# caiyuanhao1998/Open-DiffusionGS

Hardware: AMD Instinct MI355X
Metric: novel-view renders/sec (DiT step + GS raster) at 256^2 (higher is better)
Workload: dtype bf16; 1 GPU; obj-256 sampling step (BASELINE.json configs[2]): DGSDenoiser.forward = DiT image_to_gaussians (width 1024, 24 blocks, L=4098, bf16 MFMA, fp32 accumulate) + 4 fp32 rasterizations of P=262146 Gaussians at 256^2 per sample; random-init weights; batch_per_gpu=1, views=4, resolution=256, gaussians=262146, parallelism=dp1

## Files before the change

### open-diffusiongs_amd/csrc/raster_forward.hip

```cpp
#include <string.h>

#include "raster_cells.h"

namespace dgs {

struct FwdParams {
    int P, D, M, W, H, V, vps, gx, gy, T;
    const float *bg, *means3D, *shs, *colors_pre, *opac, *scales, *rots, *cov_pre, *viewm, *projm, *campos, *tanfov;
    float tanfovx, tanfovy, scale_mod;
    int prefiltered, raw_act;
    int bin_mode;
    int bitonic_cap;
    int bitonic_any;
    int exact_exp;
    int debug;
    int* radii;
    float* out_color;
    float *out_depth, *out_alpha;
    GeomState g;
    ImageState im;
    BinningState bn;
};

__device__ __forceinline__ void view_tanfov(const FwdParams& p, int v, float* tx, float* ty) {
// ... 21 lines not shown
                        -0.4570457994644658f * y * (4.0f * zz - xx - yy) * SH(11) +
                        0.3731763325901154f * z * (2.0f * zz - 3.0f * xx - 3.0f * yy) * SH(12) +
                        -0.4570457994644658f * x * (4.0f * zz - xx - yy) * SH(13) + 1.445305721320277f * z * (xx - yy) * SH(14) +
                        -0.5900435899266435f * x * (xx - 3.0f * yy) * SH(15);
                }
            }
        }
#undef SH
        r += 0.5f;
        if (r < 0) bits |= 1u << c;
        out[c] = fmaxf(r, 0.0f);
    }
    *clamp_bits = bits;
}

__device__ __forceinline__ bool preprocess_one(const FwdParams& p, int v, int idx, int* rx0, int* ry0, int* rx1, int* ry1, uint32_t* depth_key) {
    const int s = v / p.vps;
    const size_t gi = (size_t)v * p.P + idx;
    const size_t si = (size_t)s * p.P + idx;
    p.radii[gi] = 0;
    p.g.tiles_touched[gi] = 0;
    p.g.keys[0][gi] = 0xFFFFFFFFu;
    const float* vm = p.viewm + 16 * v;
    const float* pm = p.projm + 16 * v;
    const float mx = p.means3D[3 * si], my = p.means3D[3 * si + 1], mz = p.means3D[3 * si + 2];
    const float hx = pm[0] * mx + pm[4] * my + pm[8] * mz + pm[12];
    const float hy = pm[1] * mx + pm[5] * my + pm[9] * mz + pm[13];
    const float hw = pm[3] * mx + pm[7] * my + pm[11] * mz + pm[15];
    const float pw = 1.0f / (hw + 0.0000001f);
    const float projx = hx * pw, projy = hy * pw;
    float tx = vm[0] * mx + vm[4] * my + vm[8] * mz + vm[12];
    float ty = vm[1] * mx + vm[5] * my + vm[9] * mz + vm[13];
    const float tz = vm[2] * mx + vm[6] * my + vm[10] * mz + vm[14];
    if (tz <= 0.2f) {
        if (p.prefiltered) p.im.totals[1] = DGS_ERR_PREFILTERED_CULLED;
        return false;
    }
// ... 45 lines not shown
        sh_to_rgb(p.D, p.shs + 3 * (size_t)p.M * si, mx - cam[0], my - cam[1], mz - cam[2], rgb, &cbits);
    }
    float op = p.opac[si];
    if (p.raw_act) op = 1.0f / (1.0f + det_expf(-op));
    const float cut = (op > 0.0f) ? (__logf(1.0f / (255.0f * op)) - 0.004f) : __builtin_inff();
    p.g.depths[gi] = tz;
    p.radii[gi] = irad;
    p.g.means2D[gi] = make_float2(px, py);
    BlendRecord* rec = p.g.blend + gi;
    rec->co = make_float4(conx, cony, conz, op);
    rec->rc = make_float4(rgb[0], rgb[1], rgb[2], cut);
    *reinterpret_cast<float4*>(&rec->xy) = make_float4(px, py, tz, 0.f);
    p.g.clamped[gi] = (uint8_t)cbits;
    p.g.tiles_touched[gi] = (uint32_t)((y1 - y0) * (x1 - x0));
    p.g.keys[0][gi] = __float_as_uint(tz);
    *depth_key = __float_as_uint(tz);
    *rx0 = x0; *ry0 = y0; *rx1 = x1; *ry1 = y1;
    return true;
}

template <bool LDS_HIST>
__global__ __launch_bounds__(256) void preprocess_kernel(FwdParams p) {
    DGS_DYNAMIC_LDS(smem);
    uint32_t* lhist = reinterpret_cast<uint32_t*>(smem);
    const int v = blockIdx.y;
    const int idx = blockIdx.x * 256 + threadIdx.x;
    if (LDS_HIST) {
        for (int i = threadIdx.x; i < p.T; i += 256) lhist[i] = 0;
        __syncthreads();
    }
    if (blockIdx.x == 0) {
        uint32_t* w = p.g.range_ws + (size_t)v * range_ws_stride(p.P);
        for (int i = threadIdx.x; i <= kRangeBuckets; i += 256) w[i] = 0u;
    }
    int x0 = 0, y0 = 0, x1 = 0, y1 = 0;
    bool vis = false;
    uint32_t depth_key = 0xFFFFFFFFu;
    if (idx < p.P) vis = preprocess_one(p, v, idx, &x0, &y0, &x1, &y1, &depth_key);
    {
        __shared__ uint32_t s_rng[2][4];
        const uint32_t key = vis ? depth_key : 0xFFFFFFFFu;
        uint32_t hi = key != 0xFFFFFFFFu ? key : 0u, lo_c = key != 0xFFFFFFFFu ? ~key : 0u;
#pragma unroll
        for (int o = 32; o > 0; o >>= 1) { hi = max(hi, (uint32_t)__shfl_xor((int)hi, o)); lo_c = max(lo_c, (uint32_t)__shfl_xor((int)lo_c, o)); }
        if ((threadIdx.x & 63) == 0) { s_rng[0][threadIdx.x >> 6] = hi; s_rng[1][threadIdx.x >> 6] = lo_c; }
        __syncthreads();
        if (threadIdx.x < 2) {
            const uint32_t m = max(max(s_rng[threadIdx.x][0], s_rng[threadIdx.x][1]), max(s_rng[threadIdx.x][2], s_rng[threadIdx.x][3]));
            if (m) atomicMax(p.im.depth_range + ((size_t)threadIdx.x * p.V + v) * kRangeSlots + (blockIdx.x % kRangeSlots), m);
        }
    }
    uint32_t* gcount = p.im.tile_count + (size_t)v * p.T;
    if (vis) {
        uint32_t* const grid = LDS_HIST ? lhist : gcount;
        atomicAdd(&grid[y0 * p.gx + x0], 1u);
        if (x1 < p.gx) atomicAdd(&grid[y0 * p.gx + x1], 0xffffffffu);
        if (y1 < p.gy) {
            atomicAdd(&grid[y1 * p.gx + x0], 0xffffffffu);
            if (x1 < p.gx) atomicAdd(&grid[y1 * p.gx + x1], 1u);
        }
    }
    if (LDS_HIST) {
        __syncthreads();
        for (int i = threadIdx.x; i < p.T; i += 256) {
            const uint32_t c = lhist[i];
            if (c) atomicAdd(&gcount[i], c);
        }
    }
}

__global__ __launch_bounds__(256) void radix_hist_kernel(const uint32_t* keys, uint32_t* hist, int P, int NB, int shift) {
    __shared__ uint32_t h[256];
    const int v = blockIdx.y, b = blockIdx.x;
    h[threadIdx.x] = 0;
    __syncthreads();
    const uint32_t* k = keys + (size_t)v * P;
    const int base = b * kSortTile;
#pragma unroll 4
// ... 53 lines not shown
        const uint32_t rank_in_wave = (uint32_t)__popcll(peers & lt_mask);
        if (valid && rank_in_wave == 0) wcount[wave][dig] = (uint32_t)__popcll(peers);
        __syncthreads();
        if (valid) {
            uint32_t pos = running[dig] + rank_in_wave;
            for (int w = 0; w < wave; ++w) pos += wcount[w][dig];
            keys_out[vo + pos] = key;
            vals_out[vo + pos] = val;
            if (rank_of) rank_of[vo + val] = pos;
        }
        __syncthreads();
        running[tid] += wcount[0][tid] + wcount[1][tid] + wcount[2][tid] + wcount[3][tid];
    }
}

struct RangeMap {
    uint32_t lo; float scale; bool any;
    __device__ __forceinline__ uint32_t bucket(uint32_t key) const { return min((uint32_t)((float)(key - lo) * scale), (uint32_t)kRangeBuckets - 1u); }
};
__device__ __forceinline__ RangeMap range_map(const uint32_t* depth_range, int V, int v, uint32_t* s_map ) {
    if (threadIdx.x < 64) {
        const int which = threadIdx.x >> 5, slot = threadIdx.x & 31;
        uint32_t x = slot < kRangeSlots ? depth_range[((size_t)which * V + v) * kRangeSlots + slot] : 0u;
#pragma unroll
        for (int o = 16; o > 0; o >>= 1) x = max(x, (uint32_t)__shfl_xor((int)x, o));
        if (slot == 0) s_map[which] = x;
    }
    __syncthreads();
    const uint32_t hi_w = s_map[0], lo_w = s_map[1];
    const uint32_t hi = hi_w, lo = ~lo_w;
// ... 19 lines not shown
        const int i = b * kRangeTile + r * 256 + tid;
        if (i < P) {
            const uint32_t key = k[i];
            if (key != 0xFFFFFFFFu) atomicAdd(&h[m.bucket(key)], 1u); else ++culled;
        }
    }
#pragma unroll
    for (int o = 32; o > 0; o >>= 1) culled += (uint32_t)__shfl_xor((int)culled, o);
    if ((tid & 63) == 0) s_c[tid >> 6] = culled;
    __syncthreads();
    uint32_t* w = ws + (size_t)v * stride;
    for (int i = tid; i < kRangeBuckets; i += 256) { const uint32_t c = h[i]; if (c) atomicAdd(&w[i], c); }
    if (tid == 0) w[2 * kRangeBuckets + 1 + b] = (s_c[0] + s_c[1]) + (s_c[2] + s_c[3]);
}

__global__ __launch_bounds__(1024) void range_plan_kernel(uint32_t* ws, int NB, int NWIN, int stride) {
    __shared__ uint32_t scratch[20];
    __shared__ uint32_t s_start[kRangeBuckets + 1];
    uint32_t* w = ws + (size_t)blockIdx.x * stride;
    const int tid = threadIdx.x;
    const uint32_t c = tid < kRangeBuckets ? w[tid] : 0u;
    uint32_t nvis;
    const uint32_t ex = block_exclusive_scan<1024>(c, scratch, &nvis);
    __syncthreads();
    if (tid < kRangeBuckets) { w[tid] = ex; w[kRangeBuckets + 1 + tid] = 0u; s_start[tid] = ex; }
    if (tid == 0) { w[kRangeBuckets] = nvis; s_start[kRangeBuckets] = nvis; }
    __syncthreads();
    for (int j = tid; j <= NWIN; j += 1024) {
        const uint32_t want = (uint32_t)j * (uint32_t)kRangeWindow;
        int lo = 0, hi = kRangeBuckets;
        while (lo < hi) { const int mid = (lo + hi) >> 1; if (s_start[mid] < want) lo = mid + 1; else hi = mid; }
        w[2 * kRangeBuckets + 1 + NB + j] = j == NWIN ? nvis : s_start[lo];
    }
    const uint32_t cc = tid < NB ? w[2 * kRangeBuckets + 1 + tid] : 0u;
    uint32_t all;
    const uint32_t cex = block_exclusive_scan<1024>(cc, scratch, &all);
    if (tid < NB) w[2 * kRangeBuckets + 1 + tid] = nvis + cex;
}

__global__ __launch_bounds__(256) void range_scatter_kernel(const uint32_t* keys, const uint32_t* depth_range, uint32_t* ws, uint32_t* keys_out,
                                                           uint32_t* vals_out, uint32_t* order, uint32_t* rank_of, int P, int V, int stride) {
    __shared__ uint32_t h[kRangeBuckets];
    __shared__ uint32_t s_cc[kRangeItems][4];
    __shared__ uint32_t s_map[2];
    const int v = blockIdx.y, b = blockIdx.x, tid = threadIdx.x, lane = tid & 63, wave = tid >> 6;
    const RangeMap m = range_map(depth_range, V, v, s_map);
    const size_t vo = (size_t)v * P;
    uint32_t* w = ws + (size_t)v * stride;
    for (int i = tid; i < kRangeBuckets; i += 256) h[i] = 0;
    __syncthreads();
    uint32_t key[kRangeItems], slot[kRangeItems];
    const unsigned long long lt_mask = (lane == 0) ? 0ull : (~0ull >> (64 - lane));
#pragma unroll
    for (int r = 0; r < kRangeItems; ++r) {
        const int i = b * kRangeTile + r * 256 + tid;
        key[r] = i < P ? keys[vo + i] : 0u;
// ... 4 lines not shown
        if (lane == 0) s_cc[r][wave] = (uint32_t)__popcll(cm);
    }
    __syncthreads();
    {
        constexpr int Q = kRangeBuckets / 256;
        uint32_t c[Q], st0[Q], got[Q];
#pragma unroll
        for (int q = 0; q < Q; ++q) { c[q] = h[tid + 256 * q]; st0[q] = w[tid + 256 * q]; }
#pragma unroll
        for (int q = 0; q < Q; ++q) got[q] = c[q] ? atomicAdd(&w[kRangeBuckets + 1 + tid + 256 * q], c[q]) : 0u;
#pragma unroll
        for (int q = 0; q < Q; ++q) h[tid + 256 * q] = st0[q] + got[q];
    }
    __syncthreads();
    const uint32_t cbase = w[2 * kRangeBuckets + 1 + b];
#pragma unroll
    for (int r = 0; r < kRangeItems; ++r) {
        const int i = b * kRangeTile + r * 256 + tid;
        if (i >= P) continue;
        if (key[r] != 0xFFFFFFFFu) {
            const uint32_t pos = h[m.bucket(key[r])] + slot[r];
            keys_out[vo + pos] = key[r];
            vals_out[vo + pos] = (uint32_t)i;
        } else {
            uint32_t off = 0;
            for (int q = 0; q < r; ++q) off += (s_cc[q][0] + s_cc[q][1]) + (s_cc[q][2] + s_cc[q][3]);
            for (int q = 0; q < wave; ++q) off += s_cc[r][q];
            const uint32_t pos = cbase + off + slot[r];
            order[vo + pos] = (uint32_t)i;
            rank_of[vo + i] = pos;
        }
    }
}

__global__ __launch_bounds__(1024) void scan_tiles_kernel(uint32_t* count, uint2* ranges, uint32_t* cursor, int n,
                                                         int32_t* totals, long long capacity, uint32_t* order, int gx, int gy,
                                                         int32_t* stats_dev, int32_t* stats_host) {
    __shared__ uint32_t scratch[20];
    __shared__ uint32_t smax;
    __shared__ uint32_t s_class[1024];
    {
        const int T = gx * gy, V = n / T;
        for (int r = threadIdx.x; r < V * gy; r += 1024) {
            uint32_t* row = count + (size_t)(r / gy) * T + (size_t)(r % gy) * gx;
            uint32_t run = 0;
            for (int x0 = 0; x0 < gx; x0 += 16) {
                uint32_t c[16];
#pragma unroll
                for (int u = 0; u < 16; ++u) c[u] = x0 + u < gx ? row[x0 + u] : 0u;
#pragma unroll
                for (int u = 0; u < 16; ++u)
                    if (x0 + u < gx) { run += c[u]; row[x0 + u] = run; }
            }
        }
        __syncthreads();
        for (int cidx = threadIdx.x; cidx < V * gx; cidx += 1024) {
            uint32_t* col = count + (size_t)(cidx / gx) * T + (cidx % gx);
            uint32_t run = 0;
            for (int y0 = 0; y0 < gy; y0 += 16) {
                uint32_t c[16];
#pragma unroll
                for (int u = 0; u < 16; ++u) c[u] = y0 + u < gy ? col[(size_t)(y0 + u) * gx] : 0u;
#pragma unroll
                for (int u = 0; u < 16; ++u)
                    if (y0 + u < gy) { run += c[u]; col[(size_t)(y0 + u) * gx] = run; }
            }
        }
        __syncthreads();
    }
    uint32_t carry = 0, mx = 0;
    if (threadIdx.x == 0) smax = 0;
    for (int base = 0; base < n; base += 1024) {
        const int i = base + threadIdx.x;
        const uint32_t c = (i < n) ? count[i] : 0u;
        mx = max(mx, c);
        uint32_t tot;
        const uint32_t ex = block_exclusive_scan<1024>(c, scratch, &tot);
        if (i < n) { ranges[i] = make_uint2(carry + ex, carry + ex + c); cursor[i] = 0; }
        carry += tot;
    }
    __syncthreads();
    atomicMax(&smax, mx);
    __syncthreads();
    if (threadIdx.x == 0) {
        totals[0] = (int32_t)carry;
        totals[2] = (int32_t)smax;
        if (capacity >= 0 && (long long)carry > capacity) totals[1] = DGS_ERR_BINNING_OVERFLOW;
        const int32_t st1 = totals[1];
        if (stats_dev) { stats_dev[0] = (int32_t)carry; stats_dev[1] = st1; stats_dev[2] = (int32_t)smax; stats_dev[3] = 1; }
        if (stats_host) {
            stats_host[0] = (int32_t)carry; stats_host[1] = st1; stats_host[2] = (int32_t)smax;
            __threadfence_system();
            *reinterpret_cast<volatile int32_t*>(stats_host + 3) = 1;
        }
    }
    deal_tiles(count, n, smax, order, s_class, scratch);
}

enum { kFormRankSort = 1, kFormScan = 2, kFormBitonic = 3 };
__host__ __device__ __forceinline__ int binning_form_of(int bin_mode, int bitonic_cap, long long num_rendered, long long longest,
                                                        long long T, long long P, long long V, bool any_len = false) {
    const bool fits = bitonic_cap > 0 && (any_len || longest <= bitonic_cap);
    if (bin_mode == kFormScan || bin_mode == kFormRankSort) return bin_mode;
    if (bin_mode == kFormBitonic) return fits ? kFormBitonic : kFormRankSort;
    if (num_rendered * 10 >= T * P * V) return kFormScan;
    return fits ? kFormBitonic : kFormRankSort;
}
__host__ __device__ __forceinline__ bool scan_form_possible(int gx, int gy, long long T, long long P) {
    return gx <= 255 && gy <= 255 && T * P <= (1ll << 31);
}
__device__ __forceinline__ int binning_form(const FwdParams& p) {
    return binning_form_of(p.bin_mode, p.bitonic_cap, (long long)(uint32_t)p.im.totals[0], (long long)(uint32_t)p.im.totals[2], p.T, p.P, p.V,
                           p.bitonic_any != 0);
}
__device__ __forceinline__ bool binning_is_scan(const FwdParams& p) { return binning_form(p) == kFormScan; }

template <bool LDS_AGG>
__global__ __launch_bounds__(256) void emit_instances_kernel(FwdParams p) {
    DGS_DYNAMIC_LDS(smem);
    uint32_t* lcnt = reinterpret_cast<uint32_t*>(smem);
    uint32_t* lbase = lcnt + p.T;
    const int form = binning_form(p);
    if (p.im.totals[1] != 0 || form == kFormScan) return;
    const bool wide = form == kFormBitonic;
    const int v = blockIdx.y;
// ... 256 lines not shown
    }
    {
        uint32_t m = 8 * NT;
        while (m < n) m <<= 1;
        for (uint32_t i = n + tid; i < m; i += NT) keys[i] = ~0ull;
        __syncthreads();
        bitonic_sort_lds<NT>(keys, m, tid);
    }
    __syncthreads();
    for (uint32_t i = tid; i < n; i += NT) p.bn.point_list[rg.x + i] = (uint32_t)keys[i];
}

constexpr int kRangeSortCap = 8192;
template <int NT>
__global__ __launch_bounds__(NT) void range_sort_kernel(const uint32_t* ws, uint32_t* pkeys, uint32_t* pvals, uint32_t* order, uint32_t* rank_of,
                                                       int P, int stride, int seg_off) {
    DGS_DYNAMIC_LDS(smem);
    constexpr int NWV = NT / 64, KPT = kRangeSortCap / NT;
    uint64_t* keys = reinterpret_cast<uint64_t*>(smem);
    uint32_t* cnt = reinterpret_cast<uint32_t*>(smem + (size_t)kRangeSortCap * 8);
    uint32_t* cur = cnt + kBuckets;
    __shared__ uint32_t s_red[3][NWV];
    __shared__ uint32_t scratch[NWV + 4];
    const int v = blockIdx.y, tid = threadIdx.x, lane = tid & 63, wave = tid >> 6;
    const uint32_t* w = ws + (size_t)v * stride;
    const uint32_t begin = w[seg_off + blockIdx.x], end = w[seg_off + blockIdx.x + 1];
    const uint32_t n = end - begin;
    if (n == 0) return;
    const size_t vo = (size_t)v * P;
    uint32_t* pk = pkeys + vo + begin;
    uint32_t* pv = pvals + vo + begin;
    auto emit = [&](uint32_t place, uint64_t k) {
        order[vo + begin + place] = (uint32_t)k;
        rank_of[vo + (uint32_t)k] = begin + place;
    };
    if (n > (uint32_t)kRangeSortCap) {
        const uint32_t C = (uint32_t)kRangeSortCap, nchunks = (n + C - 1) / C;
        for (uint32_t c = 0; c < nchunks; ++c) {
            const uint32_t len = min(C, n - c * C);
            uint32_t m = 8 * NT;
            while (m < len) m <<= 1;
            for (uint32_t i = tid; i < m; i += NT) keys[i] = i < len ? ((uint64_t)pk[c * C + i] << 32) | pv[c * C + i] : ~0ull;
            __syncthreads();
            bitonic_sort_lds<NT>(keys, m, tid);
            __syncthreads();
            for (uint32_t i = tid; i < len; i += NT) { pk[c * C + i] = (uint32_t)(keys[i] >> 32); pv[c * C + i] = (uint32_t)keys[i]; }
            __syncthreads();
        }
        __threadfence_block();
        __syncthreads();
        for (uint32_t i = tid; i < n; i += NT) {
            const uint64_t k = ((uint64_t)pk[i] << 32) | pv[i];
            const uint32_t mine = i / C;
            uint32_t place = i - mine * C;
            for (uint32_t c = 0; c < nchunks; ++c) {
                if (c == mine) continue;
                uint32_t lo = 0, hi = min(C, n - c * C);
                while (lo < hi) {
                    const uint32_t mid = (lo + hi) >> 1;
                    const uint64_t o = ((uint64_t)pk[c * C + mid] << 32) | pv[c * C + mid];
                    if (o < k) lo = mid + 1; else hi = mid;
                }
                place += lo;
            }
            emit(place, k);
        }
        return;
    }
    uint64_t kreg[KPT];
#pragma unroll
    for (int u = 0; u < KPT; ++u) {
        const uint32_t i = (uint32_t)tid + (uint32_t)u * NT;
        kreg[u] = i < n ? ((uint64_t)pk[i] << 32) | pv[i] : ~0ull;
    }
    uint32_t lo = 0xFFFFFFFFu, hi = 0u;
#pragma unroll
    for (int u = 0; u < KPT; ++u) {
        if ((uint32_t)tid + (uint32_t)u * NT < n) {
            const uint32_t d = (uint32_t)(kreg[u] >> 32);
            lo = min(lo, d); hi = max(hi, d);
// ... 19 lines not shown
    for (uint32_t u = 0; u < per; ++u) { const uint32_t c = cnt[tid * per + u]; local += c; big = max(big, c); }
    uint32_t tot;
    uint32_t ex = block_exclusive_scan<NT>(local, scratch, &tot);
    for (uint32_t u = 0; u < per; ++u) { const uint32_t c = cnt[tid * per + u]; cur[tid * per + u] = ex; cnt[tid * per + u] = ex; ex += c; }
#pragma unroll
    for (int o = 32; o > 0; o >>= 1) big = max(big, (uint32_t)__shfl_xor((int)big, o));
    if (lane == 0) s_red[2][wave] = big;
    __syncthreads();
#pragma unroll
    for (int q = 0; q < NWV; ++q) big = max(big, s_red[2][q]);
#pragma unroll
    for (int u = 0; u < KPT; ++u)
        if ((uint32_t)tid + (uint32_t)u * NT < n) keys[atomicAdd(&cur[bucket((uint32_t)(kreg[u] >> 32))], 1u)] = kreg[u];
    __syncthreads();
    if (big <= (uint32_t)kBucketLimit) {
        for (uint32_t i = tid; i < n; i += NT) {
            const uint64_t k = keys[i];
            const uint32_t b = bucket((uint32_t)(k >> 32));
            const uint32_t s0 = cnt[b], e0 = cur[b];
            uint32_t below = 0;
            for (uint32_t j = s0; j < e0; ++j) below += keys[j] < k ? 1u : 0u;
            emit(s0 + below, k);
        }
        return;
    }
    {
        uint32_t m = 8 * NT;
        while (m < n) m <<= 1;
        for (uint32_t i = n + tid; i < m; i += NT) keys[i] = ~0ull;
        __syncthreads();
        bitonic_sort_lds<NT>(keys, m, tid);
    }
    __syncthreads();
    for (uint32_t i = tid; i < n; i += NT) emit(i, keys[i]);
}

__global__ __launch_bounds__(256) void rank_rects_kernel(FwdParams p) {
    if (p.im.totals[1] != 0 || !binning_is_scan(p)) return;
    const int v = blockIdx.y, idx = blockIdx.x * 256 + threadIdx.x;
    if (idx >= p.P) return;
    const size_t gi = (size_t)v * p.P + idx;
    uint32_t packed = 0;
    if (p.radii[gi] > 0) {
        int x0, y0, x1, y1;
        const float2 m = p.g.means2D[gi];
        tile_rect(m.x, m.y, p.radii[gi], p.gx, p.gy, &x0, &y0, &x1, &y1);
        packed = (uint32_t)x0 | ((uint32_t)y0 << 8) | ((uint32_t)x1 << 16) | ((uint32_t)y1 << 24);
    }
    p.g.vals[1][(size_t)v * p.P + p.g.rank_of[gi]] = packed;
}

constexpr uint32_t kRing = 2048;

struct TileScan {
    uint32_t next_rank;
    uint32_t found;
    uint32_t head, waiting;
};

template <bool EMIT>
__device__ __forceinline__ uint32_t scan_groups(const uint32_t* rects, const uint32_t* order, uint32_t rank_begin, int g0, int g1, uint32_t P,
                                                uint32_t tx, uint32_t ty, int lane, unsigned long long lanes_before, uint32_t off, uint32_t* ring,
                                                uint32_t ring_at, uint32_t* list, uint32_t list_at, uint32_t list_cap) {
    uint32_t cnt = 0;
// ... 295 lines not shown
    }

    const int VT = V * p.T;
    constexpr int kBitonicMax = 16384;
    static const bool lds_ok =
        hipFuncSetAttribute(reinterpret_cast<const void*>(tile_bitonic_kernel<256>), hipFuncAttributeMaxDynamicSharedMemorySize,
                            kBitonicMax * 8 + 2 * kBuckets * 4) == hipSuccess &&
        hipFuncSetAttribute(reinterpret_cast<const void*>(tile_bitonic_kernel<1024>), hipFuncAttributeMaxDynamicSharedMemorySize,
                            kBitonicMax * 8 + 2 * kBuckets * 4) == hipSuccess &&
        hipFuncSetAttribute(reinterpret_cast<const void*>(tile_bitonic_kernel<512>), hipFuncAttributeMaxDynamicSharedMemorySize,
                            kBitonicMax * 8 + 2 * kBuckets * 4) == hipSuccess &&
        hipFuncSetAttribute(reinterpret_cast<const void*>(range_sort_kernel<512>), hipFuncAttributeMaxDynamicSharedMemorySize,
                            kRangeSortCap * 8 + 2 * kBuckets * 4) == hipSuccess;
    if (!lds_ok) { fprintf(stderr, "[dgs] rasterizer: hipFuncSetAttribute(tile_bitonic_kernel, %d bytes of LDS) failed\n", kBitonicMax * 8 + 2 * kBuckets * 4); return DGS_ERR_DEVICE; }
    hipLaunchKernelGGL(zero_words_kernel, dim3(1), dim3(1024), 0, st, p.im.tile_count, (int)p.im.zero_span((size_t)V));
    const dim3 gridP((P + 255) / 256, V);
    const bool lds_tiles = p.T <= 4096;
    if (lds_tiles) hipLaunchKernelGGL((preprocess_kernel<true>), gridP, dim3(256), (size_t)p.T * 4, st, p);
    else hipLaunchKernelGGL((preprocess_kernel<false>), gridP, dim3(256), 0, st, p);
    int rc = check(st, a->debug);
    if (rc) return rc;

    const bool can_scan = scan_form_possible(p.gx, p.gy, p.T, P);
    p.bin_mode = a->binning_form;
    if (p.bin_mode < 0 || p.bin_mode > 3 || (p.bin_mode == 0 && !can_scan) || (p.bin_mode == kFormScan && !can_scan)) p.bin_mode = can_scan ? 0 : kFormBitonic;
    int bitonic_only_cap = 0;
    if (async && p.bin_mode == kFormBitonic && a->longest_hint > 0) {
        bitonic_only_cap = 2048;
        while (bitonic_only_cap < a->longest_hint + a->longest_hint / 2 && bitonic_only_cap < kBitonicMax) bitonic_only_cap <<= 1;
    }
    hipLaunchKernelGGL(scan_tiles_kernel, dim3(1), dim3(1024), 0, st, p.im.tile_count, p.im.ranges, p.im.tile_cursor, VT, p.im.totals,
                       async ? (long long)a->binning_capacity : -1LL, p.im.tile_order, p.gx, p.gy, a->num_rendered_dev, a->num_rendered_host);
    rc = check(st, a->debug);
    if (rc) return rc;

    int forms = 0;
    static thread_local int last_form = 0;
    bool radix_done = false;
    auto radix_sort = [&]() {
        const int NB = sort_blocks(P);
        static const bool use_radix = getenv("DGS_RASTER_SORT") && !strcmp(getenv("DGS_RASTER_SORT"), "radix");
        const int RB = range_blocks(P);
        if (!use_radix && RB <= 1024) {
            const int stride = (int)range_ws_stride(P);
            hipLaunchKernelGGL(range_count_kernel, dim3(RB, V), dim3(256), 0, st, p.g.keys[0], p.im.depth_range, p.g.range_ws, P, V, stride);
            const int NWIN = range_windows(P), seg_off = 2 * kRangeBuckets + 1 + RB;
            hipLaunchKernelGGL(range_plan_kernel, dim3(V), dim3(1024), 0, st, p.g.range_ws, RB, NWIN, stride);
            hipLaunchKernelGGL(range_scatter_kernel, dim3(RB, V), dim3(256), 0, st, p.g.keys[0], p.im.depth_range, p.g.range_ws, p.g.keys[1], p.g.vals[1],
                               p.g.vals[0], p.g.rank_of, P, V, stride);
            hipLaunchKernelGGL(range_sort_kernel<512>, dim3(NWIN, V), dim3(512), kRangeSortCap * 8 + 2 * kBuckets * 4, st, p.g.range_ws, p.g.keys[1], p.g.vals[1],
                               p.g.vals[0], p.g.rank_of, P, stride, seg_off);
            radix_done = true;
            return;
        }
        for (int pass = 0; pass < 4; ++pass) {
            const int in = pass & 1, out = in ^ 1;
            hipLaunchKernelGGL(radix_hist_kernel, dim3(NB, V), dim3(256), 0, st, p.g.keys[in], p.g.radix_hist, P, NB, 8 * pass);
            hipLaunchKernelGGL(radix_colscan_kernel, dim3(1, V), dim3(256), 0, st, p.g.radix_hist, p.g.radix_base, NB);
            hipLaunchKernelGGL(radix_scatter_kernel, dim3(NB, V), dim3(256), 0, st, p.g.keys[in], pass == 0 ? (const uint32_t*)nullptr : p.g.vals[in],
                               p.g.keys[out], p.g.vals[out], pass == 3 ? p.g.rank_of : (uint32_t*)nullptr, p.g.radix_hist, p.g.radix_base, P, NB, 8 * pass);
        }
        radix_done = true;
    };
    if (!async) {
        if (last_form != kFormBitonic && p.bin_mode != kFormBitonic) radix_sort();
        int32_t tot[4] = {0, 0, 0, 0};
        if (hipMemcpyAsync(tot, p.im.totals, sizeof(tot), hipMemcpyDeviceToHost, st) != hipSuccess) return DGS_ERR_DEVICE;
        if (hipStreamSynchronize(st) != hipSuccess) return DGS_ERR_DEVICE;
        if (tot[1] != 0) return tot[1];
        a->num_rendered = (int64_t)(uint32_t)tot[0];
        a->longest_list = (int64_t)(uint32_t)tot[2];
        bbuf = a->binning_alloc(dgs_raster_binning_bytes(a->num_rendered), a->binning_user);
        if (!bbuf) return DGS_ERR_ALLOC;
        p.bn = BinningState::carve(bbuf, (size_t)(a->num_rendered < 1 ? 1 : a->num_rendered), nullptr);
        int cap = 2048;
        while (cap < tot[2] && cap < kBitonicMax) cap <<= 1;
        p.bitonic_cap = cap;
        last_form = binning_form_of(p.bin_mode, p.bitonic_cap, a->num_rendered, (uint32_t)tot[2], p.T, P, V);
        forms = 1 << last_form;
    } else {
        a->num_rendered = -1;
        a->longest_list = -1;
        p.bitonic_cap = bitonic_only_cap ? bitonic_only_cap : kBitonicMax;
        p.bitonic_any = bitonic_only_cap ? 1 : 0;
        forms = p.bin_mode ? (1 << p.bin_mode) | (p.bin_mode == kFormBitonic && !bitonic_only_cap ? 1 << kFormRankSort : 0)
                           : (1 << kFormRankSort) | (1 << kFormScan) | (1 << kFormBitonic);
    }

    size_t blend_pad = 0;
    if constexpr (kRasterAblate) { static const int pad = [] { const char* e = getenv("DGS_RASTER_FWD_LDS_PAD"); return e ? atoi(e) : 0; }(); blend_pad = (size_t)pad; }
    if ((forms & ((1 << kFormRankSort) | (1 << kFormScan))) && !radix_done) radix_sort();
    if (forms & (1 << kFormScan)) {
        hipLaunchKernelGGL(rank_rects_kernel, gridP, dim3(256), 0, st, p);
        launch_blend_forward<true>(p, aux, VT, blend_pad, st);
    }
    if (forms & ((1 << kFormRankSort) | (1 << kFormBitonic))) {
        if (lds_tiles) hipLaunchKernelGGL((emit_instances_kernel<true>), gridP, dim3(256), (size_t)p.T * 8, st, p);
        else hipLaunchKernelGGL((emit_instances_kernel<false>), gridP, dim3(256), 0, st, p);
    }
    if (forms & (1 << kFormRankSort)) {
        const int wwords = pick_window_words(P);
        hipLaunchKernelGGL(tile_sort_kernel, dim3(p.T, V), dim3(256), (size_t)wwords * 4, st, p, wwords);
    }
    if (forms & (1 << kFormBitonic)) {
        const size_t lds = (size_t)p.bitonic_cap * 8 + 2 * kBuckets * 4;
        static const int nt_env = getenv("DGS_RASTER_BITONIC_NT") ? atoi(getenv("DGS_RASTER_BITONIC_NT")) : 0;
        if (p.bitonic_cap > 8192) hipLaunchKernelGGL(tile_bitonic_kernel<1024>, dim3(VT), dim3(1024), lds, st, p);
        else if (p.bitonic_cap >= 4096 && nt_env != 256) hipLaunchKernelGGL(tile_bitonic_kernel<512>, dim3(VT), dim3(512), lds, st, p);
// ... 68 lines not shown
```

### open-diffusiongs_amd/csrc/raster_state.h

```cpp
#pragma once
#include <stddef.h>
#include <stdint.h>

#include <hip/hip_runtime.h>

namespace dgs {

constexpr int kTile = 16;
constexpr int kSortItems = 16;
constexpr int kSortTile = 256 * kSortItems;
constexpr int kRangeBuckets = 1024;
constexpr int kRangeWindow = 4096;
constexpr int kRangeSlots = 16;
constexpr int kRangeItems = 8;
constexpr int kRangeTile = 256 * kRangeItems;
constexpr size_t kAlign = 256;

struct Carver {
    char* base;
    size_t off;
    explicit Carver(void* b) : base(static_cast<char*>(b)), off(0) {}
    template <class T>
    T* take(size_t count) {
        off = (off + kAlign - 1) & ~(kAlign - 1);
// ... 12 lines not shown
struct alignas(64) BlendRecord {
    float4 co;
    float4 rc;
    float2 xy;
    float z;
    float unused;
};
static_assert(sizeof(BlendRecord) == 64, "one record, one line");

struct GeomState {
    float* depths;
    float2* means2D;
    BlendRecord* blend;
    float* cov3D;
    uint8_t* clamped;
    int32_t* internal_radii;
    uint32_t* tiles_touched;
    uint32_t* keys[2];
    uint32_t* vals[2];
    uint32_t* rank_of;
    uint32_t* radix_hist;
    uint32_t* radix_base;
    uint32_t* range_ws;
    float* grad_acc;
    static GeomState carve(void* buf, size_t P, size_t V, size_t* bytes) {
        Carver c(buf);
        GeomState g;
        const size_t n = P * V;
        g.depths = c.take<float>(n);
        g.means2D = c.take<float2>(n);
        g.blend = c.take<BlendRecord>(n);
        g.cov3D = c.take<float>(6 * n);
        g.clamped = c.take<uint8_t>(n);
        g.internal_radii = c.take<int32_t>(n);
        g.tiles_touched = c.take<uint32_t>(n);
        for (int i = 0; i < 2; ++i) { g.keys[i] = c.take<uint32_t>(n); g.vals[i] = c.take<uint32_t>(n); }
        g.rank_of = c.take<uint32_t>(n);
        g.radix_hist = c.take<uint32_t>(V * (size_t)sort_blocks((int)P) * 256);
        g.radix_base = c.take<uint32_t>(V * 256);
        g.range_ws = c.take<uint32_t>(V * range_ws_stride((int)P));
        g.grad_acc = c.take<float>(16 * n);
        if (bytes) *bytes = c.bytes();
        return g;
    }
};

struct ImageState {
    float* final_T;
    uint32_t* n_contrib;
// ... 47 lines not shown
```

Before: 693.7 renders/s.

## Fuse tile scan into range plan, precompute tile rects, multi-item preprocess

Preprocess now handles four Gaussians per thread and packs each visible Gaussian's tile rectangle into a new rect_of buffer. Invisible entries are written only when culled, and the depth-range reduction runs once per block. The tile scan moves into an extra block of range_plan_kernel. The range scatter and range sort kernels write ranked rects directly when the scan form will be used, so the separate rank_rects launch and its tile_rect recomputation can be skipped. This cuts kernel launches and redundant per-Gaussian work, at the cost of extra writes inside the sort kernels and more complex ordering logic.

```diff
diff --git a/open-diffusiongs_amd/csrc/raster_forward.hip b/open-diffusiongs_amd/csrc/raster_forward.hip
--- a/open-diffusiongs_amd/csrc/raster_forward.hip
+++ b/open-diffusiongs_amd/csrc/raster_forward.hip
@@ -59,13 +59,10 @@
     *clamp_bits = bits;
 }
 
-__device__ __forceinline__ bool preprocess_one(const FwdParams& p, int v, int idx, int* rx0, int* ry0, int* rx1, int* ry1, uint32_t* depth_key) {
+__device__ __forceinline__ bool preprocess_visible(const FwdParams& p, int v, int idx, int* rx0, int* ry0, int* rx1, int* ry1, uint32_t* depth_key) {
     const int s = v / p.vps;
     const size_t gi = (size_t)v * p.P + idx;
     const size_t si = (size_t)s * p.P + idx;
-    p.radii[gi] = 0;
-    p.g.tiles_touched[gi] = 0;
-    p.g.keys[0][gi] = 0xFFFFFFFFu;
     const float* vm = p.viewm + 16 * v;
     const float* pm = p.projm + 16 * v;
     const float mx = p.means3D[3 * si], my = p.means3D[3 * si + 1], mz = p.means3D[3 * si + 2];
@@ -141,17 +138,29 @@
     p.g.clamped[gi] = (uint8_t)cbits;
     p.g.tiles_touched[gi] = (uint32_t)((y1 - y0) * (x1 - x0));
     p.g.keys[0][gi] = __float_as_uint(tz);
+    p.g.rect_of[gi] = ((uint32_t)x0 & 255u) | (((uint32_t)y0 & 255u) << 8) | (((uint32_t)x1 & 255u) << 16) | ((uint32_t)y1 << 24);
     *depth_key = __float_as_uint(tz);
     *rx0 = x0; *ry0 = y0; *rx1 = x1; *ry1 = y1;
     return true;
 }
-
+__device__ __forceinline__ bool preprocess_one(const FwdParams& p, int v, int idx, int* rx0, int* ry0, int* rx1, int* ry1, uint32_t* depth_key) {
+    const bool vis = preprocess_visible(p, v, idx, rx0, ry0, rx1, ry1, depth_key);
+    if (!vis) {
+        const size_t gi = (size_t)v * p.P + idx;
+        p.radii[gi] = 0;
+        p.g.tiles_touched[gi] = 0;
+        p.g.keys[0][gi] = 0xFFFFFFFFu;
+        p.g.rect_of[gi] = 0u;
+    }
+    return vis;
+}
+
+constexpr int kPreItems = 4, kPreTile = 256 * kPreItems;
 template <bool LDS_HIST>
 __global__ __launch_bounds__(256) void preprocess_kernel(FwdParams p) {
     DGS_DYNAMIC_LDS(smem);
     uint32_t* lhist = reinterpret_cast<uint32_t*>(smem);
     const int v = blockIdx.y;
-    const int idx = blockIdx.x * 256 + threadIdx.x;
     if (LDS_HIST) {
         for (int i = threadIdx.x; i < p.T; i += 256) lhist[i] = 0;
         __syncthreads();
@@ -160,26 +169,16 @@
         uint32_t* w = p.g.range_ws + (size_t)v * range_ws_stride(p.P);
         for (int i = threadIdx.x; i <= kRangeBuckets; i += 256) w[i] = 0u;
     }
-    int x0 = 0, y0 = 0, x1 = 0, y1 = 0;
-    bool vis = false;
-    uint32_t depth_key = 0xFFFFFFFFu;
-    if (idx < p.P) vis = preprocess_one(p, v, idx, &x0, &y0, &x1, &y1, &depth_key);
-    {
-        __shared__ uint32_t s_rng[2][4];
-        const uint32_t key = vis ? depth_key : 0xFFFFFFFFu;
-        uint32_t hi = key != 0xFFFFFFFFu ? key : 0u, lo_c = key != 0xFFFFFFFFu ? ~key : 0u;
-#pragma unroll
-        for (int o = 32; o > 0; o >>= 1) { hi = max(hi, (uint32_t)__shfl_xor((int)hi, o)); lo_c = max(lo_c, (uint32_t)__shfl_xor((int)lo_c, o)); }
-        if ((threadIdx.x & 63) == 0) { s_rng[0][threadIdx.x >> 6] = hi; s_rng[1][threadIdx.x >> 6] = lo_c; }
-        __syncthreads();
-        if (threadIdx.x < 2) {
-            const uint32_t m = max(max(s_rng[threadIdx.x][0], s_rng[threadIdx.x][1]), max(s_rng[threadIdx.x][2], s_rng[threadIdx.x][3]));
-            if (m) atomicMax(p.im.depth_range + ((size_t)threadIdx.x * p.V + v) * kRangeSlots + (blockIdx.x % kRangeSlots), m);
-        }
-    }
     uint32_t* gcount = p.im.tile_count + (size_t)v * p.T;
-    if (vis) {
-        uint32_t* const grid = LDS_HIST ? lhist : gcount;
+    uint32_t* const grid = LDS_HIST ? lhist : gcount;
+    uint32_t hi = 0u, lo_c = 0u;
+#pragma unroll 1
+    for (int r = 0; r < kPreItems; ++r) {
+        const int idx = blockIdx.x * kPreTile + r * 256 + threadIdx.x;
+        int x0 = 0, y0 = 0, x1 = 0, y1 = 0;
+        uint32_t depth_key = 0xFFFFFFFFu;
+        if (idx >= p.P || !preprocess_one(p, v, idx, &x0, &y0, &x1, &y1, &depth_key)) continue;
+        if (depth_key != 0xFFFFFFFFu) { hi = max(hi, depth_key); lo_c = max(lo_c, ~depth_key); }
         atomicAdd(&grid[y0 * p.gx + x0], 1u);
         if (x1 < p.gx) atomicAdd(&grid[y0 * p.gx + x1], 0xffffffffu);
         if (y1 < p.gy) {
@@ -187,8 +186,18 @@
             if (x1 < p.gx) atomicAdd(&grid[y1 * p.gx + x1], 1u);
         }
     }
+    {
+        __shared__ uint32_t s_rng[2][4];
+#pragma unroll
+        for (int o = 32; o > 0; o >>= 1) { hi = max(hi, (uint32_t)__shfl_xor((int)hi, o)); lo_c = max(lo_c, (uint32_t)__shfl_xor((int)lo_c, o)); }
+        if ((threadIdx.x & 63) == 0) { s_rng[0][threadIdx.x >> 6] = hi; s_rng[1][threadIdx.x >> 6] = lo_c; }
+        __syncthreads();
+        if (threadIdx.x < 2) {
+            const uint32_t m = max(max(s_rng[threadIdx.x][0], s_rng[threadIdx.x][1]), max(s_rng[threadIdx.x][2], s_rng[threadIdx.x][3]));
+            if (m) atomicMax(p.im.depth_range + ((size_t)threadIdx.x * p.V + v) * kRangeSlots + (blockIdx.x % kRangeSlots), m);
+        }
+    }
     if (LDS_HIST) {
-        __syncthreads();
         for (int i = threadIdx.x; i < p.T; i += 256) {
             const uint32_t c = lhist[i];
             if (c) atomicAdd(&gcount[i], c);
@@ -272,6 +281,29 @@
     }
 }
 
+enum { kFormRankSort = 1, kFormScan = 2, kFormBitonic = 3 };
+__host__ __device__ __forceinline__ int binning_form_of(int bin_mode, int bitonic_cap, long long num_rendered, long long longest,
+                                                        long long T, long long P, long long V, bool any_len = false) {
+    const bool fits = bitonic_cap > 0 && (any_len || longest <= bitonic_cap);
+    if (bin_mode == kFormScan || bin_mode == kFormRankSort) return bin_mode;
+    if (bin_mode == kFormBitonic) return fits ? kFormBitonic : kFormRankSort;
+    if (num_rendered * 10 >= T * P * V) return kFormScan;
+    return fits ? kFormBitonic : kFormRankSort;
+}
+__host__ __device__ __forceinline__ bool scan_form_possible(int gx, int gy, long long T, long long P) {
+    return gx <= 255 && gy <= 255 && T * P <= (1ll << 31);
+}
+struct RankRects {
+    const uint32_t* rect_of;
+    uint32_t* rects;
+    const int32_t* totals;
+    int bin_mode;
+    long long T, V;
+};
+__device__ __forceinline__ bool rank_rects_wanted(const RankRects& r, int P) {
+    return r.totals[1] == 0 && binning_form_of(r.bin_mode, 0, (long long)(uint32_t)r.totals[0], 0, r.T, P, r.V) == kFormScan;
+}
+
 struct RangeMap {
     uint32_t lo; float scale; bool any;
     __device__ __forceinline__ uint32_t bucket(uint32_t key) const { return min((uint32_t)((float)(key - lo) * scale), (uint32_t)kRangeBuckets - 1u); }
@@ -321,7 +353,79 @@
     if (tid == 0) w[2 * kRangeBuckets + 1 + b] = (s_c[0] + s_c[1]) + (s_c[2] + s_c[3]);
 }
 
-__global__ __launch_bounds__(1024) void range_plan_kernel(uint32_t* ws, int NB, int NWIN, int stride) {
+struct ScanTilesArgs {
+    uint32_t* count; uint2* ranges; uint32_t* cursor; int n;
+    int32_t* totals; long long capacity; uint32_t* order; int gx, gy;
+    int32_t *stats_dev, *stats_host;
+};
+__device__ __forceinline__ void scan_tiles(const ScanTilesArgs& a) {
+    __shared__ uint32_t scratch[20];
+    __shared__ uint32_t smax;
+    __shared__ uint32_t s_class[1024];
+    uint32_t* const count = a.count;
+    const int n = a.n, gx = a.gx, gy = a.gy;
+    const int T = gx * gy, V = n / T;
+    {
+        for (int r = threadIdx.x; r < V * gy; r += 1024) {
+            uint32_t* row = count + (size_t)(r / gy) * T + (size_t)(r % gy) * gx;
+            uint32_t run = 0;
+            for (int x0 = 0; x0 < gx; x0 += 16) {
+                uint32_t c[16];
+#pragma unroll
+                for (int u = 0; u < 16; ++u) c[u] = x0 + u < gx ? row[x0 + u] : 0u;
+#pragma unroll
+                for (int u = 0; u < 16; ++u)
+                    if (x0 + u < gx) { run += c[u]; row[x0 + u] = run; }
+            }
+        }
+        __syncthreads();
+        for (int cidx = threadIdx.x; cidx < V * gx; cidx += 1024) {
+            uint32_t* col = count + (size_t)(cidx / gx) * T + (cidx % gx);
+            uint32_t run = 0;
+            for (int y0 = 0; y0 < gy; y0 += 16) {
+                uint32_t c[16];
+#pragma unroll
+                for (int u = 0; u < 16; ++u) c[u] = y0 + u < gy ? col[(size_t)(y0 + u) * gx] : 0u;
+#pragma unroll
+                for (int u = 0; u < 16; ++u)
+                    if (y0 + u < gy) { run += c[u]; col[(size_t)(y0 + u) * gx] = run; }
+            }
+        }
+        __syncthreads();
+    }
+    uint32_t carry = 0, mx = 0;
+    if (threadIdx.x == 0) smax = 0;
+    for (int base = 0; base < n; base += 1024) {
+        const int i = base + threadIdx.x;
+        const uint32_t c = (i < n) ? count[i] : 0u;
+        mx = max(mx, c);
+        uint32_t tot;
+        const uint32_t ex = block_exclusive_scan<1024>(c, scratch, &tot);
+        if (i < n) { a.ranges[i] = make_uint2(carry + ex, carry + ex + c); a.cursor[i] = 0; }
+        carry += tot;
+    }
+    __syncthreads();
+    atomicMax(&smax, mx);
+    __syncthreads();
+    if (threadIdx.x == 0) {
+        int32_t* const totals = a.totals;
+        totals[0] = (int32_t)carry;
+        totals[2] = (int32_t)smax;
+        if (a.capacity >= 0 && (long long)carry > a.capacity) totals[1] = DGS_ERR_BINNING_OVERFLOW;
+        const int32_t st1 = totals[1];
+        if (a.stats_dev) { a.stats_dev[0] = (int32_t)carry; a.stats_dev[1] = st1; a.stats_dev[2] = (int32_t)smax; a.stats_dev[3] = 1; }
+        if (a.stats_host) {
+            a.stats_host[0] = (int32_t)carry; a.stats_host[1] = st1; a.stats_host[2] = (int32_t)smax;
+            __threadfence_system();
+            *reinterpret_cast<volatile int32_t*>(a.stats_host + 3) = 1;
+        }
+    }
+    deal_tiles(count, n, smax, a.order, s_class, scratch);
+}
+__global__ __launch_bounds__(1024) void scan_tiles_kernel(ScanTilesArgs a) { scan_tiles(a); }
+
+__global__ __launch_bounds__(1024) void range_plan_kernel(uint32_t* ws, int NB, int NWIN, int stride, int V, ScanTilesArgs tiles) {
+    if ((int)blockIdx.x == V) { scan_tiles(tiles); return; }
     __shared__ uint32_t scratch[20];
     __shared__ uint32_t s_start[kRangeBuckets + 1];
     uint32_t* w = ws + (size_t)blockIdx.x * stride;
@@ -346,7 +450,7 @@
 }
 
 __global__ __launch_bounds__(256) void range_scatter_kernel(const uint32_t* keys, const uint32_t* depth_range, uint32_t* ws, uint32_t* keys_out,
-                                                           uint32_t* vals_out, uint32_t* order, uint32_t* rank_of, int P, int V, int stride) {
+                                                           uint32_t* vals_out, uint32_t* order, uint32_t* rank_of, int P, int V, int stride, RankRects rr) {
     __shared__ uint32_t h[kRangeBuckets];
     __shared__ uint32_t s_cc[kRangeItems][4];
     __shared__ uint32_t s_map[2];
@@ -381,6 +485,7 @@
     }
     __syncthreads();
     const uint32_t cbase = w[2 * kRangeBuckets + 1 + b];
+    const bool rects = rank_rects_wanted(rr, P);
 #pragma unroll
     for (int r = 0; r < kRangeItems; ++r) {
         const int i = b * kRangeTile + r * 256 + tid;
@@ -396,86 +501,11 @@
             const uint32_t pos = cbase + off + slot[r];
             order[vo + pos] = (uint32_t)i;
             rank_of[vo + i] = pos;
-        }
-    }
-}
-
-__global__ __launch_bounds__(1024) void scan_tiles_kernel(uint32_t* count, uint2* ranges, uint32_t* cursor, int n,
-                                                         int32_t* totals, long long capacity, uint32_t* order, int gx, int gy,
-                                                         int32_t* stats_dev, int32_t* stats_host) {
-    __shared__ uint32_t scratch[20];
-    __shared__ uint32_t smax;
-    __shared__ uint32_t s_class[1024];
-    {
-        const int T = gx * gy, V = n / T;
-        for (int r = threadIdx.x; r < V * gy; r += 1024) {
-            uint32_t* row = count + (size_t)(r / gy) * T + (size_t)(r % gy) * gx;
-            uint32_t run = 0;
-            for (int x0 = 0; x0 < gx; x0 += 16) {
-                uint32_t c[16];
-#pragma unroll
-                for (int u = 0; u < 16; ++u) c[u] = x0 + u < gx ? row[x0 + u] : 0u;
-#pragma unroll
-                for (int u = 0; u < 16; ++u)
-                    if (x0 + u < gx) { run += c[u]; row[x0 + u] = run; }
-            }
-        }
-        __syncthreads();
-        for (int cidx = threadIdx.x; cidx < V * gx; cidx += 1024) {
-            uint32_t* col = count + (size_t)(cidx / gx) * T + (cidx % gx);
-            uint32_t run = 0;
-            for (int y0 = 0; y0 < gy; y0 += 16) {
-                uint32_t c[16];
-#pragma unroll
-                for (int u = 0; u < 16; ++u) c[u] = y0 + u < gy ? col[(size_t)(y0 + u) * gx] : 0u;
-#pragma unroll
-                for (int u = 0; u < 16; ++u)
-                    if (y0 + u < gy) { run += c[u]; col[(size_t)(y0 + u) * gx] = run; }
-            }
-        }
-        __syncthreads();
-    }
-    uint32_t carry = 0, mx = 0;
-    if (threadIdx.x == 0) smax = 0;
-    for (int base = 0; base < n; base += 1024) {
-        const int i = base + threadIdx.x;
-        const uint32_t c = (i < n) ? count[i] : 0u;
-        mx = max(mx, c);
-        uint32_t tot;
-        const uint32_t ex = block_exclusive_scan<1024>(c, scratch, &tot);
-        if (i < n) { ranges[i] = make_uint2(carry + ex, carry + ex + c); cursor[i] = 0; }
-        carry += tot;
-    }
-    __syncthreads();
-    atomicMax(&smax, mx);
-    __syncthreads();
-    if (threadIdx.x == 0) {
-        totals[0] = (int32_t)carry;
-        totals[2] = (int32_t)smax;
-        if (capacity >= 0 && (long long)carry > capacity) totals[1] = DGS_ERR_BINNING_OVERFLOW;
-        const int32_t st1 = totals[1];
-        if (stats_dev) { stats_dev[0] = (int32_t)carry; stats_dev[1] = st1; stats_dev[2] = (int32_t)smax; stats_dev[3] = 1; }
-        if (stats_host) {
-            stats_host[0] = (int32_t)carry; stats_host[1] = st1; stats_host[2] = (int32_t)smax;
-            __threadfence_system();
-            *reinterpret_cast<volatile int32_t*>(stats_host + 3) = 1;
-        }
-    }
-    deal_tiles(count, n, smax, order, s_class, scratch);
-}
-
-enum { kFormRankSort = 1, kFormScan = 2, kFormBitonic = 3 };
-__host__ __device__ __forceinline__ int binning_form_of(int bin_mode, int bitonic_cap, long long num_rendered, long long longest,
-                                                        long long T, long long P, long long V, bool any_len = false) {
-    const bool fits = bitonic_cap > 0 && (any_len || longest <= bitonic_cap);
-    if (bin_mode == kFormScan || bin_mode == kFormRankSort) return bin_mode;
-    if (bin_mode == kFormBitonic) return fits ? kFormBitonic : kFormRankSort;
-    if (num_rendered * 10 >= T * P * V) return kFormScan;
-    return fits ? kFormBitonic : kFormRankSort;
-}
-__host__ __device__ __forceinline__ bool scan_form_possible(int gx, int gy, long long T, long long P) {
-    return gx <= 255 && gy <= 255 && T * P <= (1ll << 31);
-}
+            if (rects) rr.rects[vo + pos] = 0u;
+        }
+    }
+}
+
 __device__ __forceinline__ int binning_form(const FwdParams& p) {
     return binning_form_of(p.bin_mode, p.bitonic_cap, (long long)(uint32_t)p.im.totals[0], (long long)(uint32_t)p.im.totals[2], p.T, p.P, p.V,
                            p.bitonic_any != 0);
@@ -762,7 +792,7 @@
 constexpr int kRangeSortCap = 8192;
 template <int NT>
 __global__ __launch_bounds__(NT) void range_sort_kernel(const uint32_t* ws, uint32_t* pkeys, uint32_t* pvals, uint32_t* order, uint32_t* rank_of,
-                                                       int P, int stride, int seg_off) {
+                                                       int P, int stride, int seg_off, RankRects rr) {
     DGS_DYNAMIC_LDS(smem);
     constexpr int NWV = NT / 64, KPT = kRangeSortCap / NT;
     uint64_t* keys = reinterpret_cast<uint64_t*>(smem);
@@ -778,9 +808,11 @@
     const size_t vo = (size_t)v * P;
     uint32_t* pk = pkeys + vo + begin;
     uint32_t* pv = pvals + vo + begin;
-    auto emit = [&](uint32_t place, uint64_t k) {
+    const bool rects = rank_rects_wanted(rr, P);
+    auto emit = [&](uint32_t place, uint64_t k, bool in_place) {
         order[vo + begin + place] = (uint32_t)k;
         rank_of[vo + (uint32_t)k] = begin + place;
+        if (in_place && rects) rr.rects[vo + begin + place] = rr.rect_of[vo + (uint32_t)k];
     };
     if (n > (uint32_t)kRangeSortCap) {
         const uint32_t C = (uint32_t)kRangeSortCap, nchunks = (n + C - 1) / C;
@@ -811,7 +843,12 @@
                 }
                 place += lo;
             }
-            emit(place, k);
+            emit(place, k, false);
+        }
+        if (rects) {
+            __threadfence_block();
+            __syncthreads();
+            for (uint32_t i = tid; i < n; i += NT) rr.rects[vo + begin + i] = rr.rect_of[vo + order[vo + begin + i]];
         }
         return;
     }
@@ -861,13 +898,23 @@
         if ((uint32_t)tid + (uint32_t)u * NT < n) keys[atomicAdd(&cur[bucket((uint32_t)(kreg[u] >> 32))], 1u)] = kreg[u];
     __syncthreads();
     if (big <= (uint32_t)kBucketLimit) {
-        for (uint32_t i = tid; i < n; i += NT) {
+        uint32_t rc[KPT];
+#pragma unroll
+        for (int u = 0; u < KPT; ++u) {
+            const uint32_t i = (uint32_t)tid + (uint32_t)u * NT;
+            rc[u] = (rects && i < n) ? rr.rect_of[vo + (uint32_t)keys[i]] : 0u;
+        }
+#pragma unroll
+        for (int u = 0; u < KPT; ++u) {
+            const uint32_t i = (uint32_t)tid + (uint32_t)u * NT;
+            if (i >= n) break;
             const uint64_t k = keys[i];
             const uint32_t b = bucket((uint32_t)(k >> 32));
             const uint32_t s0 = cnt[b], e0 = cur[b];
             uint32_t below = 0;
             for (uint32_t j = s0; j < e0; ++j) below += keys[j] < k ? 1u : 0u;
-            emit(s0 + below, k);
+            emit(s0 + below, k, false);
+            if (rects) rr.rects[vo + begin + s0 + below] = rc[u];
         }
         return;
     }
@@ -879,7 +926,7 @@
         bitonic_sort_lds<NT>(keys, m, tid);
     }
     __syncthreads();
-    for (uint32_t i = tid; i < n; i += NT) emit(i, keys[i]);
+    for (uint32_t i = tid; i < n; i += NT) emit(i, keys[i], true);
 }
 
 __global__ __launch_bounds__(256) void rank_rects_kernel(FwdParams p) {
@@ -887,14 +934,7 @@
     const int v = blockIdx.y, idx = blockIdx.x * 256 + threadIdx.x;
     if (idx >= p.P) return;
     const size_t gi = (size_t)v * p.P + idx;
-    uint32_t packed = 0;
-    if (p.radii[gi] > 0) {
-        int x0, y0, x1, y1;
-        const float2 m = p.g.means2D[gi];
-        tile_rect(m.x, m.y, p.radii[gi], p.gx, p.gy, &x0, &y0, &x1, &y1);
-        packed = (uint32_t)x0 | ((uint32_t)y0 << 8) | ((uint32_t)x1 << 16) | ((uint32_t)y1 << 24);
-    }
-    p.g.vals[1][(size_t)v * p.P + p.g.rank_of[gi]] = packed;
+    p.g.vals[1][(size_t)v * p.P + p.g.rank_of[gi]] = p.g.rect_of[gi];
 }
 
 constexpr uint32_t kRing = 2048;
@@ -1220,10 +1260,10 @@
                             kRangeSortCap * 8 + 2 * kBuckets * 4) == hipSuccess;
     if (!lds_ok) { fprintf(stderr, "[dgs] rasterizer: hipFuncSetAttribute(tile_bitonic_kernel, %d bytes of LDS) failed\n", kBitonicMax * 8 + 2 * kBuckets * 4); return DGS_ERR_DEVICE; }
     hipLaunchKernelGGL(zero_words_kernel, dim3(1), dim3(1024), 0, st, p.im.tile_count, (int)p.im.zero_span((size_t)V));
-    const dim3 gridP((P + 255) / 256, V);
+    const dim3 gridP((P + 255) / 256, V), gridPre((P + kPreTile - 1) / kPreTile, V);
     const bool lds_tiles = p.T <= 4096;
-    if (lds_tiles) hipLaunchKernelGGL((preprocess_kernel<true>), gridP, dim3(256), (size_t)p.T * 4, st, p);
-    else hipLaunchKernelGGL((preprocess_kernel<false>), gridP, dim3(256), 0, st, p);
+    if (lds_tiles) hipLaunchKernelGGL((preprocess_kernel<true>), gridPre, dim3(256), (size_t)p.T * 4, st, p);
+    else hipLaunchKernelGGL((preprocess_kernel<false>), gridPre, dim3(256), 0, st, p);
     int rc = check(st, a->debug);
     if (rc) return rc;
 
@@ -1235,10 +1275,13 @@
         bitonic_only_cap = 2048;
         while (bitonic_only_cap < a->longest_hint + a->longest_hint / 2 && bitonic_only_cap < kBitonicMax) bitonic_only_cap <<= 1;
     }
-    hipLaunchKernelGGL(scan_tiles_kernel, dim3(1), dim3(1024), 0, st, p.im.tile_count, p.im.ranges, p.im.tile_cursor, VT, p.im.totals,
-                       async ? (long long)a->binning_capacity : -1LL, p.im.tile_order, p.gx, p.gy, a->num_rendered_dev, a->num_rendered_host);
-    rc = check(st, a->debug);
-    if (rc) return rc;
+    const ScanTilesArgs tiles{p.im.tile_count, p.im.ranges, p.im.tile_cursor, VT, p.im.totals, async ? (long long)a->binning_capacity : -1LL,
+                              p.im.tile_order, p.gx, p.gy, a->num_rendered_dev, a->num_rendered_host};
+    bool tiles_scanned = false, rects_ranked = false;
+    auto scan_tiles_now = [&]() {
+        if (!tiles_scanned) hipLaunchKernelGGL(scan_tiles_kernel, dim3(1), dim3(1024), 0, st, tiles);
+        tiles_scanned = true;
+    };
 
     int forms = 0;
     static thread_local int last_form = 0;
@@ -1251,14 +1294,17 @@
             const int stride = (int)range_ws_stride(P);
             hipLaunchKernelGGL(range_count_kernel, dim3(RB, V), dim3(256), 0, st, p.g.keys[0], p.im.depth_range, p.g.range_ws, P, V, stride);
             const int NWIN = range_windows(P), seg_off = 2 * kRangeBuckets + 1 + RB;
-            hipLaunchKernelGGL(range_plan_kernel, dim3(V), dim3(1024), 0, st, p.g.range_ws, RB, NWIN, stride);
+            hipLaunchKernelGGL(range_plan_kernel, dim3(V + (tiles_scanned ? 0 : 1)), dim3(1024), 0, st, p.g.range_ws, RB, NWIN, stride, V, tiles);
+            tiles_scanned = true;
+            const RankRects rr{p.g.rect_of, p.g.vals[1], p.im.totals, p.bin_mode, (long long)p.T, (long long)V};
             hipLaunchKernelGGL(range_scatter_kernel, dim3(RB, V), dim3(256), 0, st, p.g.keys[0], p.im.depth_range, p.g.range_ws, p.g.keys[1], p.g.vals[1],
-                               p.g.vals[0], p.g.rank_of, P, V, stride);
+                               p.g.vals[0], p.g.rank_of, P, V, stride, rr);
             hipLaunchKernelGGL(range_sort_kernel<512>, dim3(NWIN, V), dim3(512), kRangeSortCap * 8 + 2 * kBuckets * 4, st, p.g.range_ws, p.g.keys[1], p.g.vals[1],
-                               p.g.vals[0], p.g.rank_of, P, stride, seg_off);
-            radix_done = true;
+                               p.g.vals[0], p.g.rank_of, P, stride, seg_off, rr);
+            radix_done = rects_ranked = true;
             return;
         }
+        scan_tiles_now();
         for (int pass = 0; pass < 4; ++pass) {
             const int in = pass & 1, out = in ^ 1;
             hipLaunchKernelGGL(radix_hist_kernel, dim3(NB, V), dim3(256), 0, st, p.g.keys[in], p.g.radix_hist, P, NB, 8 * pass);
@@ -1270,6 +1316,9 @@
     };
     if (!async) {
         if (last_form != kFormBitonic && p.bin_mode != kFormBitonic) radix_sort();
+        scan_tiles_now();
+        rc = check(st, a->debug);
+        if (rc) return rc;
         int32_t tot[4] = {0, 0, 0, 0};
         if (hipMemcpyAsync(tot, p.im.totals, sizeof(tot), hipMemcpyDeviceToHost, st) != hipSuccess) return DGS_ERR_DEVICE;
         if (hipStreamSynchronize(st) != hipSuccess) return DGS_ERR_DEVICE;
@@ -1291,13 +1340,17 @@
         p.bitonic_any = bitonic_only_cap ? 1 : 0;
         forms = p.bin_mode ? (1 << p.bin_mode) | (p.bin_mode == kFormBitonic && !bitonic_only_cap ? 1 << kFormRankSort : 0)
                            : (1 << kFormRankSort) | (1 << kFormScan) | (1 << kFormBitonic);
+        if (forms & ((1 << kFormRankSort) | (1 << kFormScan))) radix_sort();
+        scan_tiles_now();
+        rc = check(st, a->debug);
+        if (rc) return rc;
     }
 
     size_t blend_pad = 0;
     if constexpr (kRasterAblate) { static const int pad = [] { const char* e = getenv("DGS_RASTER_FWD_LDS_PAD"); return e ? atoi(e) : 0; }(); blend_pad = (size_t)pad; }
     if ((forms & ((1 << kFormRankSort) | (1 << kFormScan))) && !radix_done) radix_sort();
     if (forms & (1 << kFormScan)) {
-        hipLaunchKernelGGL(rank_rects_kernel, gridP, dim3(256), 0, st, p);
+        if (!rects_ranked) hipLaunchKernelGGL(rank_rects_kernel, gridP, dim3(256), 0, st, p);
         launch_blend_forward<true>(p, aux, VT, blend_pad, st);
     }
     if (forms & ((1 << kFormRankSort) | (1 << kFormBitonic))) {
diff --git a/open-diffusiongs_amd/csrc/raster_state.h b/open-diffusiongs_amd/csrc/raster_state.h
--- a/open-diffusiongs_amd/csrc/raster_state.h
+++ b/open-diffusiongs_amd/csrc/raster_state.h
@@ -50,7 +50,7 @@
     BlendRecord* blend;
     float* cov3D;
     uint8_t* clamped;
-    int32_t* internal_radii;
+    uint32_t* rect_of;
     uint32_t* tiles_touched;
     uint32_t* keys[2];
     uint32_t* vals[2];
@@ -68,7 +68,7 @@
         g.blend = c.take<BlendRecord>(n);
         g.cov3D = c.take<float>(6 * n);
         g.clamped = c.take<uint8_t>(n);
-        g.internal_radii = c.take<int32_t>(n);
+        g.rect_of = c.take<uint32_t>(n);
         g.tiles_touched = c.take<uint32_t>(n);
         for (int i = 0; i < 2; ++i) { g.keys[i] = c.take<uint32_t>(n); g.vals[i] = c.take<uint32_t>(n); }
         g.rank_of = c.take<uint32_t>(n);
```

Measured after the change: 696.1 renders/s, median of 5. No clear change (+0.3%).
